# VITA-Group/mm-hand

Measured on AMD Instinct MI355X. Metric: 256x256 hand images/sec (G+D step), higher is better.
Workload: dtype f32; 1 GPU; RHD-shaped 256x256, per-GPU batch 32, fp32 (Winograd F(6x6,3x3) on the 3x3 stack), G(9 PATBlocks, ngf64)+D_PB+D_PP+L1/perceptual/GAN+Adam, --norm instance, dropout on; VGG19[:4] weights: random-init (seed 1234): NOT the reference's pretrained objective; global_batch=32, parallelism=dp1

## Files before the change

### mmhand_amd/csrc/common.h

```cpp
#pragma once
#include <hip/hip_runtime.h>
#include <cstdarg>
#include <cstdio>
#include <cstdint>
#include "../../include/mmhand_hip.h"

namespace mmh {

char* err_buf();
int fail(const char* fmt, ...);

inline int check_launch(const char* what) {
    hipError_t e = hipGetLastError();
    if (e != hipSuccess) return fail("%s: %s", what, hipGetErrorString(e));
    return 0;
}

inline hipStream_t as_stream(mmh_stream_t s) { return reinterpret_cast<hipStream_t>(s); }

inline int64_t cdiv(int64_t a, int64_t b) { return (a + b - 1) / b; }

int wino6_weights(const float* w, float* U, int Cin, int Cout, int flip_transpose, hipStream_t st);
int wino6_weights_multi(const long long* table, int n, long long total_blocks, hipStream_t st);
int wino6_input(const float* x, float* V, int B, int H, int W, int C, int reflect, int xcd, hipStream_t st);
int wino6_output(const float* M, float* y, const float* bias, int B, int H, int W, int C, int act, float* stats,
                 int fold, hipStream_t st);
int wino6_dy(const float* dy, float* Yh, int B, int H, int W, int C, hipStream_t st);
int wino6_input_normact(const float* x, float* V, int B, int H, int W, int C, int reflect, int xcd,
                        const float* scale, const float* shift, int groups, int relu, float drop_p,
                        const uint32_t* drows, hipStream_t st);
int wino6_input_dy_normbwd(const float* g, const float* x, float* V, float* Yh, int B, int H, int W, int C, int xcd,
                           int fold, const float* mean, const float* invstd, const float* gamma, const float* s1,
                           const float* s2, double count, const float* scale, const float* shift,
                           const uint32_t* drows, int groups, int relu, float drop_p, hipStream_t st);
int wino6_input_dy(const float* dy, float* V, float* Yh, int B, int H, int W, int C, int xcd, int fold,
                   hipStream_t st);
int wino6_dw(const float* dU, float* dw, int Cin, int Cout, int accumulate, hipStream_t st);
bool wgrad_lp16t_supported(const mmh_conv_desc* d);
int wgrad_lp16t_splits(const mmh_conv_desc* d);
int launch_wgrad_lp16t(const mmh_conv_desc* d, const void* x16, const void* dy16, float* slab, const void* zeros,
                       hipStream_t st);
bool dgrad_s2_halo_ok(const mmh_conv_desc* d, int dx_cs, int act);
int launch_dgrad_s2_halo(const mmh_conv_desc* d, const void* dy, const void* w, const void* bias, void* dx, int dx_cs,
                         int act, hipStream_t st);
extern int g_dgrad_s2_halo, g_dgrad_s2_dbg;
bool wgrad_s2_strip_ok(const mmh_conv_desc* d);
size_t wgrad_s2_strip_ws_bytes(const mmh_conv_desc* d);
int launch_wgrad_s2_strip(const mmh_conv_desc* d, const void* x, const void* dy, void* dw, void* ws, size_t ws_bytes,
                          int accumulate, hipStream_t st);
extern int g_wgrad_s2_strip;
bool stem_f32_ok(const mmh_conv_desc* d);
int stem_f32_stats_chunks(const mmh_conv_desc* d);
int launch_stem_f32(const mmh_conv_desc* d, const void* x, const void* w, const void* bias, void* y, int act, float* stats,
                    hipStream_t st);
extern int g_stem_f32, g_stem_f32_dbg, g_stem_f32_levels;
extern int g_stem_sparse;
extern int g_stem_sparse_flat;
void wgrad_flat_split(int Mrows, int N, int P, int& splits, int& pix_per_split);
bool wino_wgrad_dma_ok(int64_t tiles, int Cin, int Cout, int nbatch);
size_t wino_wgrad_dma_ws_bytes(int64_t tiles, int Cin, int Cout, int nbatch);
int launch_wino_wgrad_dma(const float* V, const float* Yh, int64_t tiles, int Cin, int Cout, int nbatch, float* ws, float* dU,
                          hipStream_t st);
extern int g_wino_wgrad_dma;
int launch_slab_reduce(const float* slab, float* dw, int64_t n4_total, int splits, int accumulate, int64_t n4, hipStream_t st);
bool conv_s2f_ok(const mmh_conv_desc* d, int mode);
bool conv_s1f_ok(const mmh_conv_desc* d, int mode);
int conv_s2f_stats_chunks(const mmh_conv_desc* d);
int launch_conv_s2f(const mmh_conv_desc* d, const void* x16, const void* w16, const void* bias, void* y, int y_is16, int act,
                    const void* zeros, hipStream_t st, float* stats = nullptr, int mode = 0);
bool conv_s2d_ok(const mmh_conv_desc* d, int mode);
int launch_conv_s2d(const mmh_conv_desc* d, const void* g16, const void* w16, const void* bias, void* dx, int dx_is16, int act,
                    const void* zeros, hipStream_t st);
extern int g_lp16_s2f;
extern int g_lp16_persist;
extern int g_slab_reduce_par;
extern int g_wino6_vec;
extern int g_lp16_shape;
extern int g_lp16_tap_inner;
extern int g_lp16_dbg;
extern int g_lp16_wgrad_ring;
extern int g_lp16_wgrad_s2;
extern int g_pw_v2;
extern int g_col_chunks, g_row_chunks;

}

#define MMH_REQUIRE(cond, ...)                      \
    do {                                            \
        if (!(cond)) return mmh::fail(__VA_ARGS__); \
    } while (0)
// ... 1 lines not shown
```

### mmhand_amd/csrc/conv_igemm.hip

```cpp
#include <algorithm>
#include <cstring>
#include "device_prims.h"

namespace {
using namespace mmh::dev;

typedef __bf16 bf16x4 __attribute__((ext_vector_type(4)));
typedef __bf16 bf16x2 __attribute__((ext_vector_type(2)));
typedef _Float16 f16x4 __attribute__((ext_vector_type(4)));
typedef _Float16 f16x2 __attribute__((ext_vector_type(2)));
__device__ __forceinline__ bf16x4 to_bf16x4(float4 v) {
    bf16x4 r;
    r[0] = (__bf16)v.x; r[1] = (__bf16)v.y; r[2] = (__bf16)v.z; r[3] = (__bf16)v.w;
    return r;
}
template <bool H16>
__device__ __forceinline__ bf16x4 to_lp4(float4 v) {
    if (H16) {
        f16x4 r;
        r[0] = (_Float16)v.x; r[1] = (_Float16)v.y; r[2] = (_Float16)v.z; r[3] = (_Float16)v.w;
        return __builtin_bit_cast(bf16x4, r);
    }
    return to_bf16x4(v);
}
// ... 2179 lines not shown

Gather fwd_gather(const mmh_conv_desc* d, const void* x) {
    Gather g{};
    g.src = static_cast<const float*>(x);
    g.src_bytes = (unsigned)((size_t)d->B * d->H * d->W * d->x_cs * sizeof(float));
    g.srcH = d->H; g.srcW = d->W; g.src_cs = (unsigned)d->x_cs;
    g.PH = d->Ho; g.PW = d->Wo;
    g.TH = d->kh; g.TW = d->kw;
    g.C4 = d->Cin / 4;
    g.ap_h = d->stride; g.at_h = 1; g.a0_h = -d->pad;
    g.ap_w = d->stride; g.at_w = 1; g.a0_w = -d->pad;
    g.shift = 0;
    g.reflect = d->pad_mode == MMH_PAD_REFLECT;
    return g;
}

int fprop_stats_chunks(const mmh_conv_desc* d) {
    if (mmh::stem_f32_ok(d)) return mmh::stem_f32_stats_chunks(d);
    const long long M = (long long)d->B * d->Ho * d->Wo;
    if (is16(d->dtype) || M % BM != 0 || d->Cout % 4 != 0) return 0;
    const int waves_m = d->Cout > 32 ? 2 : 4;
    return (int)(M / BM) * waves_m;
}

int do_fprop(const mmh_conv_desc* d, const void* x, const void* w, const void* bias, void* y,
             int act, hipStream_t st, float* stats = nullptr, const int* rect_pads = nullptr) {
    if (!rect_pads && mmh::stem_f32_ok(d) && (!stats || mmh::stem_f32_stats_chunks(d) > 0))
        return mmh::launch_stem_f32(d, x, w, bias, y, act, stats, st);
    ConvKP p{};
    p.stats = stats;
    p.g = fwd_gather(d, x);
    if (rect_pads) { p.g.a0_h = -rect_pads[0]; p.g.a0_w = -rect_pads[1]; }
    set_korder(p.g, p.nk, p.Kflat);
    p.w = static_cast<const float*>(w);
    p.w_bytes = (unsigned)((size_t)d->kh * d->kw * d->Cin * d->Cout * sizeof(float));
    p.out = static_cast<float*>(y);
    p.bias = static_cast<const float*>(bias);
    p.M = d->B * d->Ho * d->Wo;
    p.N = d->Cout;
    p.wCin = d->Cin; p.wCout = d->Cout;
    p.KW_true = d->kw; p.kh0 = 0; p.kw0 = 0; p.tstep = 1;
    p.out_linear = 1; p.out_cs = (unsigned)d->y_cs;
    p.OH = d->Ho; p.OW = d->Wo; p.o_p = 1;
    p.act = act;
    if (is16(d->dtype)) {
        p.h16 = d->dtype == MMH_FP16;
        if (d->Cin % 64 == 0) {
            p.wRows = d->Cout; p.wKper = d->Cin;
            p.w_bytes = (unsigned)((size_t)d->kh * d->kw * d->Cin * d->Cout * 2);
        } else {
            const int Kpad = (d->kh * d->kw * d->Cin + 63) / 64 * 64;
            p.flat16 = 1;
            p.wRows = d->Cout; p.wKper = Kpad;
            p.w_bytes = (unsigned)((size_t)d->Cout * Kpad * 2);
        }
        return launch_conv_bf16(p, st);
    }
    return launch_conv<false>(p, st);
}

int g_dgrad_s2_multi = 1;
template <int BN, int WM, int WN, int BMT = 128>
int launch_multi_t(MultiKP& mp, bool bf16, hipStream_t st);

int do_dgrad(const mmh_conv_desc* d, const void* dy, const void* w, const void* bias, void* dx,
             int dx_cs, int act, hipStream_t st) {
// ... 676 lines not shown
}

struct OptionEntry { const char* name; int* value; };
const OptionEntry* option_table(int* count) {
    static const OptionEntry table[] = {
        {"conv_dbuf", &g_conv_dbuf},
        {"conv_dbg", &g_conv_dbg},
        {"conv_cw", &g_conv_cw},
        {"conv_bn256", &g_conv_bn256},
        {"conv_levels", &g_conv_levels},
        {"dgrad_levels", &g_dgrad_levels},
        {"wino_bn256", &g_wino_bn256},
        {"conv_xcd", &g_conv_xcd},
        {"conv_xcd1", &g_conv_xcd1},
        {"conv_tall", &g_conv_tall},
        {"wgrad_slots", &g_wgrad_slots},
        {"wgrad_dbuf", &g_wgrad_dbuf},
        {"wgrad_bn256", &g_wgrad_bn256},
        {"wgrad_xcd", &g_wgrad_xcd},
        {"wino_wgrad_v2", &g_wino_wgrad_v2},
        {"wino_wgrad_occ", &g_wino_wgrad_occ},
        {"wino_gemm_v2", &g_wino_gemm_v2},
        {"wino_xcd", &g_wino_xcd},
        {"dgrad_s2_multi", &g_dgrad_s2_multi},
        {"wino6_vec", &mmh::g_wino6_vec},
        {"lp16_shape", &mmh::g_lp16_shape},
        {"lp16_s2f", &mmh::g_lp16_s2f},
        {"lp16_persist", &mmh::g_lp16_persist},
        {"lp16_tap_inner", &mmh::g_lp16_tap_inner},
        {"pw_v2", &mmh::g_pw_v2},
        {"col_chunks", &mmh::g_col_chunks},
        {"row_chunks", &mmh::g_row_chunks},
        {"dgrad_s2_halo", &mmh::g_dgrad_s2_halo},
        {"wgrad_s2_strip", &mmh::g_wgrad_s2_strip},
        {"stem_f32", &mmh::g_stem_f32},
        {"wino_wgrad_dma", &mmh::g_wino_wgrad_dma},
        {"stem_f32_dbg", &mmh::g_stem_f32_dbg},
        {"slab_reduce_par", &mmh::g_slab_reduce_par},
        {"dgrad_s2_dbg", &mmh::g_dgrad_s2_dbg},
        {"lp16_dbg", &mmh::g_lp16_dbg},
        {"lp16_wgrad_ring", &mmh::g_lp16_wgrad_ring},
        {"lp16_wgrad_s2", &mmh::g_lp16_wgrad_s2},
        {"border_bn64", &g_border_bn64},
        {"wino_gemm_occ", &g_wino_gemm_occ},
        {"wino_gemm_levels", &g_wino_gemm_levels},
        {"wino_gemm_bn", &g_wino_gemm_bn},
        {"wino_bf16_occ", &g_wino_bf16_occ},
        {"wino_bf16_bk", &g_wino_bf16_bk},
        {"wino_wgrad_bn256", &g_wino_wgrad_bn256},
        {"wino_wgrad_slots", &g_wino_wgrad_slots},
        {"stem_sparse", &mmh::g_stem_sparse},
        {"stem_sparse_flat", &mmh::g_stem_sparse_flat},
    };
    *count = (int)(sizeof(table) / sizeof(table[0]));
    return table;
}
const OptionEntry* find_option(const char* key) {
    int n = 0;
    const OptionEntry* t = option_table(&n);
    for (int i = 0; i < n; ++i)
        if (!strcmp(key, t[i].name)) return &t[i];
    return nullptr;
}

}

namespace mmh {
void wgrad_flat_split(int Mrows, int N, int P, int& splits, int& pix_per_split) {
    splits = wgrad_splits(Mrows, N, P);
    pix_per_split = wgrad_pix_per_split(P, splits, BK);
}
}

extern "C" {

int mmh_set_option(const char* key, int value) {
    MMH_REQUIRE(key != nullptr, "mmh_set_option: NULL key");
    const OptionEntry* e = find_option(key);
    if (!e) return mmh::fail("mmh_set_option: unknown key '%s'", key);
    if (e->value == &g_conv_levels) { g_conv_levels = value == 2 ? 2 : 1; mmh::g_stem_f32_levels = g_conv_levels; return 0; }
    if (e->value == &g_dgrad_levels) { g_dgrad_levels = value == 2 ? 2 : 1; return 0; }
    if (e->value == &mmh::g_col_chunks || e->value == &mmh::g_row_chunks)
        MMH_REQUIRE(value > 0, "mmh_set_option: '%s' needs a value > 0, got %d", key, value);
    *e->value = value;
    return 0;
// ... 506 lines not shown
```

### mmhand_amd/csrc/conv_thin.hip

```cpp
#include <algorithm>
#include "device_prims.h"

namespace {
using namespace mmh::dev;

constexpr int TW = 64, TH = 16;
constexpr int HC = TW + 6, HR = TH + 6;
constexpr unsigned OOBT = 0xFFFFFFF0u;

typedef float f2 __attribute__((ext_vector_type(2)));
typedef unsigned u4 __attribute__((ext_vector_type(4)));

struct ThinKP {
    const float* x;
    unsigned x_bytes;
    int B, H, W, Cin, x_cs;
    const float* w;
    const float* bias;
    float* y;
    int Ho, Wo, y_cs;
    int pad, reflect, act;
    int tiles_x, tiles_y;
    int x_lp;
};

__global__ void __launch_bounds__(256) thin_conv7_kernel(const ThinKP p) {
    __shared__ float4 xs[HR * HC];
    const int tid = threadIdx.x;
    const int lane = tid & 63, wave = tid >> 6;
    int t = blockIdx.x;
    const int tx = t % p.tiles_x; t /= p.tiles_x;
    const int ty = t % p.tiles_y;
    const int b = t / p.tiles_y;
    const int oh0 = ty * TH, ow0 = tx * TW;
    const __amdgpu_buffer_rsrc_t rs =
        __builtin_amdgcn_make_buffer_rsrc(const_cast<float*>(p.x), 0, p.x_bytes, 0x00020000);

    constexpr int NLD = (HR * HC + 255) / 256;
    unsigned soff[NLD];
#pragma unroll
    for (int i = 0; i < NLD; ++i) {
        const int idx = tid + 256 * i;
        const int r = idx / HC, c = idx - r * HC;
        int ih = oh0 + r - p.pad, iw = ow0 + c - p.pad;
        bool ok = idx < HR * HC;
        if (p.reflect) {
            ih = ih < 0 ? -ih : ih;
            iw = iw < 0 ? -iw : iw;
            ih = ih >= p.H ? 2 * (p.H - 1) - ih : ih;
            iw = iw >= p.W ? 2 * (p.W - 1) - iw : iw;
            ok = ok && ih >= 0 && iw >= 0 && ih < p.H && iw < p.W;
        } else {
            ok = ok && ih >= 0 && iw >= 0 && ih < p.H && iw < p.W;
        }
        soff[i] = ok ? (unsigned)(((b * p.H + ih) * p.W + iw) * p.x_cs) * (p.x_lp ? 2u : 4u) : OOBT;
    }

    f2 acc[4][2];
#pragma unroll
    for (int q = 0; q < 4; ++q) { acc[q][0] = (f2){0.f, 0.f}; acc[q][1] = (f2){0.f, 0.f}; }

    for (int c0 = 0; c0 < p.Cin; c0 += 4) {
        float4 st[NLD];
#pragma unroll
        for (int i = 0; i < NLD; ++i) {
            if (p.x_lp) {
                typedef unsigned u2 __attribute__((ext_vector_type(2)));
                const u2 v = __builtin_amdgcn_raw_buffer_load_b64(rs, soff[i] == OOBT ? OOBT : soff[i] + c0 * 2u, 0, 0);
                if (p.x_lp == 1) {
                    st[i] = make_float4(__uint_as_float(v[0] << 16), __uint_as_float(v[0] & 0xffff0000u),
                                        __uint_as_float(v[1] << 16), __uint_as_float(v[1] & 0xffff0000u));
                } else {
                    auto h = [](unsigned bits) { return (float)__builtin_bit_cast(_Float16, (unsigned short)bits); };
                    st[i] = make_float4(h(v[0] & 0xffffu), h(v[0] >> 16), h(v[1] & 0xffffu), h(v[1] >> 16));
                }
            } else {
                const u4 v = __builtin_amdgcn_raw_buffer_load_b128(rs, soff[i] == OOBT ? OOBT : soff[i] + c0 * 4u, 0, 0);
                st[i] = __builtin_bit_cast(float4, v);
            }
        }
        __syncthreads();
#pragma unroll
        for (int i = 0; i < NLD; ++i)
            if (tid + 256 * i < HR * HC) xs[tid + 256 * i] = st[i];
        __syncthreads();
        const float* wc = p.w + c0 * 4;
#pragma unroll 1
        for (int kw = 0; kw < 7; ++kw) {
            float4 xv[10];
// ... 5 lines not shown
                f2 w01[4], w23[4];
#pragma unroll
                for (int ci = 0; ci < 4; ++ci) {
                    w01[ci] = (f2){wt[ci * 4 + 0], wt[ci * 4 + 1]};
                    w23[ci] = (f2){wt[ci * 4 + 2], wt[ci * 4 + 3]};
                }
#pragma unroll
                for (int q = 0; q < 4; ++q) {
                    const float4 xx = xv[q + kh];
                    const float xc[4] = {xx.x, xx.y, xx.z, xx.w};
#pragma unroll
                    for (int ci = 0; ci < 4; ++ci) {
                        const f2 xb = (f2){xc[ci], xc[ci]};
                        acc[q][0] = __builtin_elementwise_fma(xb, w01[ci], acc[q][0]);
                        acc[q][1] = __builtin_elementwise_fma(xb, w23[ci], acc[q][1]);
                    }
                }
            }
        }
    }

    float bs[4] = {0.f, 0.f, 0.f, 0.f};
    if (p.bias) { bs[0] = p.bias[0]; bs[1] = p.bias[1]; bs[2] = p.bias[2]; bs[3] = p.bias[3]; }
    const int ow = ow0 + lane;
#pragma unroll
    for (int q = 0; q < 4; ++q) {
        const int oh = oh0 + wave * 4 + q;
        if (oh < p.Ho && ow < p.Wo) {
            float4 o;
            o.x = act_apply(acc[q][0].x + bs[0], p.act);
            o.y = act_apply(acc[q][0].y + bs[1], p.act);
            o.z = act_apply(acc[q][1].x + bs[2], p.act);
            o.w = act_apply(acc[q][1].y + bs[3], p.act);
            *reinterpret_cast<float4*>(p.y + ((size_t)(b * p.Ho + oh) * p.Wo + ow) * p.y_cs) = o;
        }
    }
}

__global__ void thin_flip_weights_kernel(const float* __restrict__ w, int wCin, int Cout, float* __restrict__ wq) {
    const int i = blockIdx.x * blockDim.x + threadIdx.x;
    if (i >= 49 * Cout * 4) return;
    const int j = i & 3;
    const int co = (i >> 2) % Cout;
    const int tap = (i >> 2) / Cout;
    const int kh = tap / 7, kw = tap - kh * 7;
    wq[i] = j < wCin ? w[(((6 - kh) * 7 + (6 - kw)) * wCin + j) * Cout + co] : 0.f;
}

__global__ void thin_reflect_fold_kernel(const float* __restrict__ dxp, float* __restrict__ dx, int B, int H, int W,
                                         int dx_cs, int p) {
    const long long total = (long long)B * H * W;
    long long i = (long long)blockIdx.x * blockDim.x + threadIdx.x;
    const long long stride = (long long)gridDim.x * blockDim.x;
    const int HP = H + 2 * p, WP = W + 2 * p;
    for (; i < total; i += stride) {
        const int w = (int)(i % W);
        const long long t = i / W;
        const int h = (int)(t % H);
        const int b = (int)(t / H);
        int hs[3], ws[3], nh = 0, nw = 0;
        hs[nh++] = h + p;
        if (h >= 1 && h <= p) hs[nh++] = p - h;
        if (h <= H - 2 && h >= H - 1 - p) hs[nh++] = 2 * (H - 1) - h + p;
        ws[nw++] = w + p;
        if (w >= 1 && w <= p) ws[nw++] = p - w;
        if (w <= W - 2 && w >= W - 1 - p) ws[nw++] = 2 * (W - 1) - w + p;
        float4 s = make_float4(0.f, 0.f, 0.f, 0.f);
        for (int a = 0; a < nh; ++a)
            for (int c = 0; c < nw; ++c) {
                const float4 v = *reinterpret_cast<const float4*>(dxp + ((size_t)(b * HP + hs[a]) * WP + ws[c]) * 4);
                s.x += v.x; s.y += v.y; s.z += v.z; s.w += v.w;
            }
        *reinterpret_cast<float4*>(dx + (size_t)i * dx_cs) = s;
    }
}

constexpr int WGW = 32;
constexpr int WGC = WGW + 6;

struct ThinWgKP {
    const float* x;
    unsigned x_bytes;
    const float* dy;
    unsigned dy_bytes;
    float* slab;
    int B, H, W, Cin, x_cs, dy_cs, reflect;
    int strips, chunks;
    int segs, seg_rows;
};

__global__ void __launch_bounds__(448) thin_wgrad7_kernel(const ThinWgKP p) {
    __shared__ float ring[8][WGC][64];
    __shared__ float4 dyrow[2][WGW];
    const int tid = threadIdx.x;
    const int lane = tid & 63, kh = tid >> 6;
    int t = blockIdx.x;
    const int chunk = t % p.chunks; t /= p.chunks;
    const int strip = t % p.strips; t /= p.strips;
    const int seg = t % p.segs;
    const int b = t / p.segs;
    const int r0 = seg * p.seg_rows, r1 = min(p.H, r0 + p.seg_rows);
    const int w0 = strip * WGW;
    const __amdgpu_buffer_rsrc_t rsx = __builtin_amdgcn_make_buffer_rsrc(const_cast<float*>(p.x), 0, p.x_bytes, 0x00020000);
    const __amdgpu_buffer_rsrc_t rsd = __builtin_amdgcn_make_buffer_rsrc(const_cast<float*>(p.dy), 0, p.dy_bytes, 0x00020000);

    constexpr int NF4 = WGC * 16;
    auto row_off = [&](int ir, int idx) -> unsigned {
        const int px = idx >> 4, c4 = idx & 15;
        int iw = w0 + px - 3;
        bool ok = idx < NF4;
        if (p.reflect) {
            ir = ir < 0 ? -ir : ir; ir = ir >= p.H ? 2 * (p.H - 1) - ir : ir;
            iw = iw < 0 ? -iw : iw; iw = iw >= p.W ? 2 * (p.W - 1) - iw : iw;
        }
        ok = ok && ir >= 0 && ir < p.H && iw >= 0 && iw < p.W;
        return ok ? (unsigned)(((b * p.H + ir) * p.W + iw) * p.x_cs + chunk * 64 + c4 * 4) * 4u : OOBT;
    };
    float4 st[2];
    float4 sd = make_float4(0.f, 0.f, 0.f, 0.f);
    auto load_row = [&](int ir, int orow) {
#pragma unroll
        for (int i = 0; i < 2; ++i) {
            const u4 v = __builtin_amdgcn_raw_buffer_load_b128(rsx, row_off(ir, tid + 448 * i), 0, 0);
            st[i] = __builtin_bit_cast(float4, v);
        }
        if (tid < WGW) {
            const int ow = w0 + tid;
            const unsigned off = (orow < p.H && ow < p.W) ? (unsigned)(((b * p.H + orow) * p.W + ow) * p.dy_cs) * 4u : OOBT;
            sd = __builtin_bit_cast(float4, __builtin_amdgcn_raw_buffer_load_b128(rsd, off, 0, 0));
        }
    };
    auto store_row = [&](int ir, int orow) {
        float* slot = &ring[(ir + 3) & 7][0][0];
#pragma unroll
        for (int i = 0; i < 2; ++i) {
            const int idx = tid + 448 * i;
            if (idx < NF4) *reinterpret_cast<float4*>(slot + (idx >> 4) * 64 + (idx & 15) * 4) = st[i];
        }
        if (tid < WGW) dyrow[orow & 1][tid] = sd;
    };

    f2 acc[7][2];
#pragma unroll
    for (int k = 0; k < 7; ++k) { acc[k][0] = (f2){0.f, 0.f}; acc[k][1] = (f2){0.f, 0.f}; }

    for (int ir = r0 - 3; ir <= r0 + 2; ++ir) { load_row(ir, p.H); store_row(ir, r0 + 1); }
    load_row(r0 + 3, r0);
    store_row(r0 + 3, r0);
    __syncthreads();
    for (int r = r0; r < r1; ++r) {
        if (r + 1 < r1) load_row(r + 4, r + 1);
        const float* xr = &ring[(r + kh) & 7][0][lane];
        float xv[WGC];
#pragma unroll
        for (int c = 0; c < WGC; ++c) xv[c] = xr[c * 64];
#pragma unroll
        for (int c = 0; c < WGW; ++c) {
            const float4 d4 = dyrow[r & 1][c];
            const f2 d01 = (f2){d4.x, d4.y}, d23 = (f2){d4.z, d4.w};
#pragma unroll
            for (int kw = 0; kw < 7; ++kw) {
                const f2 xb = (f2){xv[c + kw], xv[c + kw]};
                acc[kw][0] = __builtin_elementwise_fma(xb, d01, acc[kw][0]);
                acc[kw][1] = __builtin_elementwise_fma(xb, d23, acc[kw][1]);
            }
        }
        if (r + 1 < r1) store_row(r + 4, r + 1);
        __syncthreads();
    }
    float* out = p.slab + ((size_t)blockIdx.x * 49 + kh * 7) * 256 + lane * 4;
#pragma unroll
    for (int kw = 0; kw < 7; ++kw)
        *reinterpret_cast<float4*>(out + kw * 256) = make_float4(acc[kw][0].x, acc[kw][0].y, acc[kw][1].x, acc[kw][1].y);
}

__global__ void thin_wgrad_reduce_kernel(const float* __restrict__ slab, float* __restrict__ dw, int nbs, int chunks,
                                         int Cin, int accumulate) {
    const int i = blockIdx.x * blockDim.x + threadIdx.x;
    if (i >= 49 * Cin) return;
    const int tap = i / Cin, ci = i - tap * Cin;
    const int chunk = ci >> 6, cl = ci & 63;
    float4 s = make_float4(0.f, 0.f, 0.f, 0.f);
    for (int k = 0; k < nbs; ++k) {
        const float4 v = *reinterpret_cast<const float4*>(slab + (((size_t)(k * chunks + chunk) * 49 + tap) * 64 + cl) * 4);
        s.x += v.x; s.y += v.y; s.z += v.z; s.w += v.w;
    }
    float4* o = reinterpret_cast<float4*>(dw) + i;
    if (accumulate) { const float4 v = *o; s.x += v.x; s.y += v.y; s.z += v.z; s.w += v.w; }
    *o = s;
}

int launch_thin(ThinKP& p, hipStream_t st) {
    p.tiles_x = (p.Wo + TW - 1) / TW;
    p.tiles_y = (p.Ho + TH - 1) / TH;
    const long long blocks = (long long)p.B * p.tiles_x * p.tiles_y;
    MMH_REQUIRE(blocks > 0 && blocks < (1ll << 31), "thin conv: grid too large");
    hipLaunchKernelGGL(thin_conv7_kernel, dim3((unsigned)blocks), dim3(256), 0, st, p);
    return mmh::check_launch("thin_conv7_kernel");
}

bool thin_shape_ok(const mmh_conv_desc* d) {
    return d && d->kh == 7 && d->kw == 7 && d->stride == 1 && d->pad == 3 && d->dtype == MMH_F32 && d->B > 0 &&
           d->H > 3 && d->W > 3 && d->Ho == d->H && d->Wo == d->W;
}

}

extern "C" {

int mmh_conv7_thin_fprop(const mmh_conv_desc* d, const void* x, const void* w, const void* bias, void* y, int act,
                         mmh_stream_t s) {
    MMH_REQUIRE(thin_shape_ok(d), "mmh_conv7_thin_fprop: needs a 7x7 / stride 1 / pad 3 fp32 conv");
    MMH_REQUIRE(d->Cout == 4 && d->Cin % 4 == 0 && d->Cin > 0 && d->x_cs >= d->Cin && d->x_cs % 4 == 0 &&
                    d->y_cs >= 4 && d->y_cs % 4 == 0,
                "mmh_conv7_thin_fprop: needs Cout == 4 (3 padded to 4) and channel counts %% 4 == 0");
    MMH_REQUIRE(x && w && y, "mmh_conv7_thin_fprop: NULL buffer");
    const long long xb = (long long)d->B * d->H * d->W * d->x_cs * 4;
    MMH_REQUIRE(xb < (1ll << 32) - 64, "mmh_conv7_thin_fprop: input too large for 32-bit offsets");
    ThinKP p{};
    p.x = static_cast<const float*>(x); p.x_bytes = (unsigned)xb;
    p.B = d->B; p.H = d->H; p.W = d->W; p.Cin = d->Cin; p.x_cs = d->x_cs;
    p.w = static_cast<const float*>(w); p.bias = static_cast<const float*>(bias);
    p.y = static_cast<float*>(y); p.Ho = d->Ho; p.Wo = d->Wo; p.y_cs = d->y_cs;
    p.pad = 3; p.reflect = d->pad_mode == MMH_PAD_REFLECT; p.act = act;
    return launch_thin(p, mmh::as_stream(s));
}

size_t mmh_conv7_thin_dgrad_ws_bytes(const mmh_conv_desc* d) {
    if (!thin_shape_ok(d)) return 0;
// ... 44 lines not shown
static int thin_wg_segs(const mmh_conv_desc* d) {
    const long long base = (long long)d->B * ((d->W + WGW - 1) / WGW) * (d->Cin / 64);
    const long long want = (256 + base - 1) / base;
    return (int)std::max<long long>(1, std::min<long long>(want, d->H / 32));
}

size_t mmh_conv7_thin_wgrad_ws_bytes(const mmh_conv_desc* d) {
    if (!thin_shape_ok(d) || d->Cin % 64) return 0;
    const size_t nblk = (size_t)d->B * ((d->W + WGW - 1) / WGW) * (d->Cin / 64) * thin_wg_segs(d);
    return nblk * 49 * 64 * 4 * sizeof(float);
}

int mmh_conv7_thin_wgrad(const mmh_conv_desc* d, const void* x, const void* dy, void* dw, void* ws, size_t ws_bytes,
                         int accumulate, mmh_stream_t s) {
    MMH_REQUIRE(thin_shape_ok(d), "mmh_conv7_thin_wgrad: needs a 7x7 / stride 1 / pad 3 fp32 conv");
    MMH_REQUIRE(d->Cout == 4 && d->Cin % 64 == 0 && d->Cin > 0 && d->x_cs >= d->Cin && d->x_cs % 4 == 0 && d->y_cs >= 4 &&
                    d->y_cs % 4 == 0,
                "mmh_conv7_thin_wgrad: needs Cout == 4 and Cin %% 64 == 0");
    MMH_REQUIRE(x && dy && dw && ws && ws_bytes >= mmh_conv7_thin_wgrad_ws_bytes(d), "mmh_conv7_thin_wgrad: bad buffers");
    const long long xb = (long long)d->B * d->H * d->W * d->x_cs * 4, yb = (long long)d->B * d->H * d->W * d->y_cs * 4;
    MMH_REQUIRE(xb < (1ll << 32) - 64 && yb < (1ll << 32) - 64, "mmh_conv7_thin_wgrad: tensors too large for 32-bit offsets");
    hipStream_t st = mmh::as_stream(s);
    ThinWgKP p{};
    p.x = static_cast<const float*>(x); p.x_bytes = (unsigned)xb;
    p.dy = static_cast<const float*>(dy); p.dy_bytes = (unsigned)yb;
    p.slab = static_cast<float*>(ws);
    p.B = d->B; p.H = d->H; p.W = d->W; p.Cin = d->Cin; p.x_cs = d->x_cs; p.dy_cs = d->y_cs;
    p.reflect = d->pad_mode == MMH_PAD_REFLECT;
    p.strips = (d->W + WGW - 1) / WGW;
    p.chunks = d->Cin / 64;
    p.segs = thin_wg_segs(d);
    p.seg_rows = (d->H + p.segs - 1) / p.segs;
    const int nblk = d->B * p.segs * p.strips * p.chunks;
    hipLaunchKernelGGL(thin_wgrad7_kernel, dim3(nblk), dim3(448), 0, st, p);
    if (int rc = mmh::check_launch("thin_wgrad7_kernel")) return rc;
    const int n4 = 49 * d->Cin;
    hipLaunchKernelGGL(thin_wgrad_reduce_kernel, dim3((n4 + 255) / 256), dim3(256), 0, st, p.slab, static_cast<float*>(dw),
                       d->B * p.segs * p.strips, p.chunks, d->Cin, accumulate);
    return mmh::check_launch("thin_wgrad_reduce_kernel");
}

}
```

Measured before the change: 129.4 images/s.

## Add persistent XCD-aware MFMA kernel for stride-2 3x3 f32 forward convs

Adds a dedicated persistent kernel for the generator's stride-2 3x3 downsampling convolutions (64->128, 128->256) in fp32. It uses a three-stage LDS DMA pipeline, zero-line halo handling and fp32 32x32x2 MFMA, and fuses bias plus instance-norm statistics into the epilogue. The epilogue of each tile overlaps with loads for the next one. It replaces the generic implicit-GEMM path for these shapes when there is no activation. Risks are heavy LDS use at one block per CU and possible stats-layout mismatch with the generic path.

```diff
diff --git a/mmhand_amd/csrc/common.h b/mmhand_amd/csrc/common.h
--- a/mmhand_amd/csrc/common.h
+++ b/mmhand_amd/csrc/common.h
@@ -44,6 +44,10 @@
 int launch_dgrad_s2_halo(const mmh_conv_desc* d, const void* dy, const void* w, const void* bias, void* dx, int dx_cs,
                          int act, hipStream_t st);
 extern int g_dgrad_s2_halo, g_dgrad_s2_dbg;
+bool fprop_s2_ok(const mmh_conv_desc* d);
+int launch_fprop_s2(const mmh_conv_desc* d, const void* x, const void* w, const void* bias, void* y, float* stats,
+                    hipStream_t st);
+extern int g_fprop_s2_halo;
 bool wgrad_s2_strip_ok(const mmh_conv_desc* d);
 size_t wgrad_s2_strip_ws_bytes(const mmh_conv_desc* d);
 int launch_wgrad_s2_strip(const mmh_conv_desc* d, const void* x, const void* dy, void* dw, void* ws, size_t ws_bytes,
diff --git a/mmhand_amd/csrc/conv_igemm.hip b/mmhand_amd/csrc/conv_igemm.hip
--- a/mmhand_amd/csrc/conv_igemm.hip
+++ b/mmhand_amd/csrc/conv_igemm.hip
@@ -2235,6 +2235,8 @@
     p.g = fwd_gather(d, x);
     if (rect_pads) { p.g.a0_h = -rect_pads[0]; p.g.a0_w = -rect_pads[1]; }
     set_korder(p.g, p.nk, p.Kflat);
+    if (!rect_pads && act == MMH_ACT_NONE && g_conv_levels == 1 && p.g.chunk_major && p.g.cw == 2 && mmh::fprop_s2_ok(d))
+        return mmh::launch_fprop_s2(d, x, w, bias, y, stats, st);
     p.w = static_cast<const float*>(w);
     p.w_bytes = (unsigned)((size_t)d->kh * d->kw * d->Cin * d->Cout * sizeof(float));
     p.out = static_cast<float*>(y);
@@ -2977,6 +2979,7 @@
         {"col_chunks", &mmh::g_col_chunks},
         {"row_chunks", &mmh::g_row_chunks},
         {"dgrad_s2_halo", &mmh::g_dgrad_s2_halo},
+        {"fprop_s2_halo", &mmh::g_fprop_s2_halo},
         {"wgrad_s2_strip", &mmh::g_wgrad_s2_strip},
         {"stem_f32", &mmh::g_stem_f32},
         {"wino_wgrad_dma", &mmh::g_wino_wgrad_dma},
diff --git a/mmhand_amd/csrc/fprop_s2.hip b/mmhand_amd/csrc/fprop_s2.hip
--- /dev/null
+++ b/mmhand_amd/csrc/fprop_s2.hip
@@ -0,0 +1,275 @@
+#include <algorithm>
+#include <type_traits>
+#include "device_prims.h"
+
+namespace mmh { int g_fprop_s2_halo = 1; }
+
+namespace {
+using namespace mmh::dev;
+
+constexpr int NT = 512;
+constexpr int BMT = 128;
+constexpr int KP = 32;
+constexpr int NST = 3;
+constexpr int A_B = BMT * KP * 4;
+constexpr int b_bytes(int tn) { return KP * 128 * tn * 4; }
+constexpr int stage_bytes(int tn) { return A_B + b_bytes(tn); }
+constexpr int lds_bytes(int tn) { return NST * stage_bytes(tn); }
+
+__device__ __attribute__((aligned(128))) char g_zero_line[128];
+constexpr int wait_vm(int n) { return (n & 15) | ((n >> 4) << 14) | 0x0070; }
+template <int V> using IC = std::integral_constant<int, V>;
+
+struct FpropS2KP {
+    const float* x;
+    const float* w;
+    const float* bias;
+    float* y;
+    float* stats;
+    int H, W, Ho, Wo, x_cs, y_cs;
+    int tiles, per_xcd, slots;
+};
+
+template <int TN>
+__global__ void __launch_bounds__(NT, 1) fprop_s2_kernel(const FpropS2KP p) {
+    constexpr int N = 128 * TN, CIN = 64 * TN, SC = TN;
+    constexpr int B_B = b_bytes(TN), STAGE = stage_bytes(TN);
+    constexpr int BR = B_B / (NT * 16);
+    constexpr int NI = 2 + BR;
+    constexpr int CPR = N / 4;
+    constexpr int RPR = NT / CPR;
+    extern __shared__ __attribute__((aligned(1024))) char smem[];
+    const int tid = threadIdx.x;
+    const int lane = tid & 63, wave = __builtin_amdgcn_readfirstlane(tid >> 6);
+    const int l31 = lane & 31, h = lane >> 5;
+    const int wm = wave >> 2, wn = wave & 3;
+    const unsigned lds0 = lds_addr_of(smem);
+    const unsigned wdst = __builtin_amdgcn_readfirstlane(lds0 + (unsigned)wave * 1024u);
+    const int xcd = blockIdx.x & 7, slot = blockIdx.x >> 3;
+    const int t_end = min(p.tiles, (xcd + 1) * p.per_xcd);
+    int tile = xcd * p.per_xcd + slot;
+    if (tile >= t_end) return;
+
+    const int ncol = wn * 32 * TN + l31;
+    float bv[TN];
+#pragma unroll
+    for (int j = 0; j < TN; ++j) {
+        bv[j] = p.bias ? p.bias[ncol + 32 * j] : 0.f;
+        asm volatile("" : "+v"(bv[j]));
+    }
+
+    const int arow = tid >> 3;
+    const unsigned a_coff = (unsigned)(((tid & 7) ^ ((tid >> 4) & 7)) << 2);
+    const unsigned w_lane_off = (unsigned)(((tid / CPR) * N + ((tid % CPR) << 2)) * 4);
+    const int HoWo = p.Ho * p.Wo;
+    int ptile = tile, psc = 0, pkh = 0, pkw = 0, pj = 0;
+    int a_pix[2];
+    bool a_top[2], a_left[2];
+    auto set_ptile = [&]() {
+#pragma unroll
+        for (int rr = 0; rr < 2; ++rr) {
+            const int m = ptile * BMT + rr * 64 + arow;
+            const int b = m / HoWo;
+            const int rem = m - b * HoWo;
+            const int oh = rem / p.Wo, ow = rem - (rem / p.Wo) * p.Wo;
+            a_pix[rr] = (b * p.H + 2 * oh - 1) * p.W + 2 * ow - 1;
+            a_top[rr] = oh == 0;
+            a_left[rr] = ow == 0;
+        }
+    };
+    auto issue = [&](int stage) {
+        const bool live = ptile < t_end;
+        const int c0 = psc * 64 + pj * KP;
+        const unsigned dst = wdst + (unsigned)(stage * STAGE);
+#pragma unroll
+        for (int rr = 0; rr < 2; ++rr) {
+            const bool ok = live && !(pkh == 0 && a_top[rr]) && !(pkw == 0 && a_left[rr]);
+            const int pix = ok ? a_pix[rr] + pkh * p.W + pkw : 0;
+            const void* g = ok ? (const void*)(p.x + (size_t)pix * (size_t)p.x_cs + c0 + a_coff)
+                               : (const void*)(g_zero_line + (lane & 7) * 16);
+            lds_dma16(g, dst + (unsigned)(rr * NT * 16));
+        }
+        const float* src = p.w + (size_t)((pkh * 3 + pkw) * CIN + c0) * N;
+#pragma unroll
+        for (int rr = 0; rr < BR; ++rr) dma16_s(src + rr * RPR * N, w_lane_off, dst + (unsigned)(A_B + rr * NT * 16));
+        if (++pj == 2) {
+            pj = 0;
+            if (++pkw == 3) {
+                pkw = 0;
+                if (++pkh == 3) {
+                    pkh = 0;
+                    if (++psc == SC) { psc = 0; ptile += p.slots; set_ptile(); }
+                }
+            }
+        }
+    };
+
+    const unsigned a_lane = lds0 + (unsigned)((wm * 64 + l31) * (KP * 4)) + (unsigned)((h ^ ((l31 >> 1) & 7)) << 4);
+    const unsigned b_lane = lds0 + (unsigned)A_B + (unsigned)((h * 4 * N + ncol) * 4);
+    f32x16 acc[2][TN];
+
+    auto epilogue = [&](int t) {
+        float* const yo = p.y + (size_t)(t * BMT + wm * 64) * (size_t)p.y_cs + ncol;
+#pragma unroll
+        for (int i = 0; i < 2; ++i)
+#pragma unroll
+            for (int r = 0; r < 16; ++r) {
+                const int m = i * 32 + (r & 3) + 8 * (r >> 2) + 4 * h;
+#pragma unroll
+                for (int j = 0; j < TN; ++j) yo[(size_t)m * (size_t)p.y_cs + 32 * j] = acc[i][j][r] + bv[j];
+            }
+        if (p.stats) {
+            constexpr float CNT = 32.f;
+#pragma unroll
+            for (int j = 0; j < TN; ++j) {
+                const float b = bv[j];
+                float sum = 0.f;
+#pragma unroll
+                for (int i = 0; i < 2; ++i)
+#pragma unroll
+                    for (int r = 0; r < 16; ++r) sum += acc[i][j][r] + b;
+                const float mean_l = sum * (1.f / CNT);
+                float m2 = 0.f;
+#pragma unroll
+                for (int i = 0; i < 2; ++i)
+#pragma unroll
+                    for (int r = 0; r < 16; ++r) {
+                        const float dv = acc[i][j][r] + b - mean_l;
+                        m2 += dv * dv;
+                    }
+                const float mean_o = __shfl_xor(mean_l, 32, 64), m2_o = __shfl_xor(m2, 32, 64);
+                const float dm = mean_o - mean_l;
+                if (h == 0) {
+                    float* o = p.stats + ((size_t)(t * 2 + wm) * 3) * N + ncol + 32 * j;
+                    o[0] = 2.f * CNT;
+                    o[N] = mean_l + 0.5f * dm;
+                    o[2 * N] = m2 + m2_o + dm * dm * (0.5f * CNT);
+                }
+            }
+        }
+    };
+
+    int prev = -1;
+    auto phase = [&](auto phc, bool first) {
+        constexpr int ph = decltype(phc)::value;
+        constexpr int S = ph % NST, SN = (ph + 2) % NST;
+        asm volatile("" ::: "memory");
+        if (ph == 1 && first && prev >= 0) __builtin_amdgcn_s_waitcnt(wait_vm(0));
+        else __builtin_amdgcn_s_waitcnt(wait_vm(NI));
+        __builtin_amdgcn_s_barrier();
+        asm volatile("" ::: "memory");
+        issue(SN);
+        if (ph == 0 && first) {
+            if (prev >= 0) epilogue(prev);
+#pragma unroll
+            for (int i = 0; i < 2; ++i)
+#pragma unroll
+                for (int j = 0; j < TN; ++j)
+#pragma unroll
+                    for (int r = 0; r < 16; ++r) acc[i][j][r] = 0.f;
+        }
+        unsigned ab = a_lane + (unsigned)(S * STAGE), bb = b_lane + (unsigned)(S * STAGE);
+        asm volatile("" : "+v"(ab), "+v"(bb));
+        f32x4 af[2];
+        float bf[TN][4];
+#pragma unroll
+        for (int i = 0; i < 2; ++i) af[i] = lds_f4(ab, i * 32 * KP * 4);
+#pragma unroll
+        for (int j = 0; j < TN; ++j)
+#pragma unroll
+            for (int e = 0; e < 4; ++e) bf[j][e] = lds_f(bb, (e * N + 32 * j) * 4);
+#pragma unroll
+        for (int kg = 0; kg < 4; ++kg) {
+            f32x4 an[2];
+            float bn[TN][4];
+            if (kg + 1 < 4) {
+#pragma unroll
+                for (int i = 0; i < 2; ++i) an[i] = lds_f4(ab ^ (unsigned)((kg + 1) << 5), i * 32 * KP * 4);
+#pragma unroll
+                for (int j = 0; j < TN; ++j)
+#pragma unroll
+                    for (int e = 0; e < 4; ++e) bn[j][e] = lds_f(bb, (((kg + 1) * 8 + e) * N + 32 * j) * 4);
+            }
+#pragma unroll
+            for (int e = 0; e < 4; ++e)
+#pragma unroll
+                for (int i = 0; i < 2; ++i)
+#pragma unroll
+                    for (int j = 0; j < TN; ++j)
+                        acc[i][j] = __builtin_amdgcn_mfma_f32_32x32x2f32(af[i][e], bf[j][e], acc[i][j], 0, 0, 0);
+            if (kg + 1 < 4) {
+#pragma unroll
+                for (int i = 0; i < 2; ++i) af[i] = an[i];
+#pragma unroll
+                for (int j = 0; j < TN; ++j)
+#pragma unroll
+                    for (int e = 0; e < 4; ++e) bf[j][e] = bn[j][e];
+            }
+        }
+    };
+
+    set_ptile();
+    issue(0);
+    issue(1);
+    for (; tile < t_end; tile += p.slots) {
+        for (int sc = 0; sc < SC; ++sc)
+            for (int kh = 0; kh < 3; ++kh) {
+                const bool first = sc == 0 && kh == 0;
+                phase(IC<0>{}, first); phase(IC<1>{}, first); phase(IC<2>{}, first);
+                phase(IC<3>{}, first); phase(IC<4>{}, first); phase(IC<5>{}, first);
+            }
+        prev = tile;
+    }
+    epilogue(prev);
+    __builtin_amdgcn_s_waitcnt(wait_vm(0));
+}
+
+}
+
+namespace mmh {
+
+bool fprop_s2_ok(const mmh_conv_desc* d) {
+    return g_fprop_s2_halo && d->dtype == MMH_F32 && d->kh == 3 && d->kw == 3 && d->stride == 2 && d->pad == 1 &&
+           d->pad_mode == MMH_PAD_ZERO && ((d->Cin == 64 && d->Cout == 128) || (d->Cin == 128 && d->Cout == 256)) &&
+           d->H == 2 * d->Ho && d->W == 2 * d->Wo && ((long long)d->B * d->Ho * d->Wo) % BMT == 0 &&
+           d->x_cs >= d->Cin && d->x_cs % 4 == 0 && d->y_cs >= d->Cout &&
+           (long long)d->B * d->H * d->W * d->x_cs < (1ll << 31) && (long long)d->B * d->Ho * d->Wo * d->y_cs < (1ll << 31);
+}
+
+template <int TN>
+static int launch_t(const FpropS2KP& p, hipStream_t st) {
+    static int ready = -1;
+    if (ready != 0) {
+        hipError_t e = hipFuncSetAttribute(reinterpret_cast<const void*>(fprop_s2_kernel<TN>),
+                                           hipFuncAttributeMaxDynamicSharedMemorySize, lds_bytes(TN));
+        if (e != hipSuccess) return fail("fprop_s2: %s", hipGetErrorString(e));
+        ready = 0;
+    }
+    hipLaunchKernelGGL((fprop_s2_kernel<TN>), dim3(8 * p.slots), dim3(NT), lds_bytes(TN), st, p);
+    return check_launch("fprop_s2_kernel");
+}
+
+int launch_fprop_s2(const mmh_conv_desc* d, const void* x, const void* w, const void* bias, void* y, float* stats,
+                    hipStream_t st) {
+    FpropS2KP p{};
+    p.x = static_cast<const float*>(x);
+    p.w = static_cast<const float*>(w);
+    p.bias = static_cast<const float*>(bias);
+    p.y = static_cast<float*>(y);
+    p.stats = stats;
+    p.H = d->H; p.W = d->W; p.Ho = d->Ho; p.Wo = d->Wo; p.x_cs = d->x_cs; p.y_cs = d->y_cs;
+    p.tiles = (int)((long long)d->B * d->Ho * d->Wo / BMT);
+    p.per_xcd = (p.tiles + 7) / 8;
+    static int cus = 0;
+    if (!cus) {
+        int dev = 0;
+        hipDeviceProp_t prop;
+        if (hipGetDevice(&dev) != hipSuccess || hipGetDeviceProperties(&prop, dev) != hipSuccess)
+            return fail("fprop_s2: cannot query the device");
+        cus = prop.multiProcessorCount;
+    }
+    p.slots = std::max(1, std::min(cus / 8, p.per_xcd));
+    return d->Cin == 64 ? launch_t<1>(p, st) : launch_t<2>(p, st);
+}
+
+}
```

Measured after the change: 130.1 images/s (median of 6 runs). About the same (+0.6%).

## Use 4x4x1 f32 MFMA broadcast for thin 7x7 conv fprop and wgrad

Applied to the files above, without the earlier changes.

Adds MFMA variants of the thin 7x7 Cout=4 convolution forward and weight-gradient kernels. Both use the 4x4x1 f32 matrix instruction in broadcast mode to replace scalar FMA chains. The forward kernel restructures staging to 16-channel groups with a register prefetch of the next group's weights and input. The new path is on by default behind a thin_mfma option, but the forward MFMA path runs only for fp32 input. It raises register pressure through the 49-entry weight double buffer and triples shared memory in fprop, and these kernels are a small part of the full G+D step.

```diff
diff --git a/mmhand_amd/csrc/common.h b/mmhand_amd/csrc/common.h
--- a/mmhand_amd/csrc/common.h
+++ b/mmhand_amd/csrc/common.h
@@ -56,6 +56,7 @@
 extern int g_stem_f32, g_stem_f32_dbg, g_stem_f32_levels;
 extern int g_stem_sparse;
 extern int g_stem_sparse_flat;
+extern int g_thin_mfma;
 void wgrad_flat_split(int Mrows, int N, int P, int& splits, int& pix_per_split);
 bool wino_wgrad_dma_ok(int64_t tiles, int Cin, int Cout, int nbatch);
 size_t wino_wgrad_dma_ws_bytes(int64_t tiles, int Cin, int Cout, int nbatch);
diff --git a/mmhand_amd/csrc/conv_igemm.hip b/mmhand_amd/csrc/conv_igemm.hip
--- a/mmhand_amd/csrc/conv_igemm.hip
+++ b/mmhand_amd/csrc/conv_igemm.hip
@@ -2996,6 +2996,7 @@
         {"wino_wgrad_slots", &g_wino_wgrad_slots},
         {"stem_sparse", &mmh::g_stem_sparse},
         {"stem_sparse_flat", &mmh::g_stem_sparse_flat},
+        {"thin_mfma", &mmh::g_thin_mfma},
     };
     *count = (int)(sizeof(table) / sizeof(table[0]));
     return table;
diff --git a/mmhand_amd/csrc/conv_thin.hip b/mmhand_amd/csrc/conv_thin.hip
--- a/mmhand_amd/csrc/conv_thin.hip
+++ b/mmhand_amd/csrc/conv_thin.hip
@@ -1,5 +1,8 @@
 #include <algorithm>
+#include <type_traits>
 #include "device_prims.h"
+
+namespace mmh { int g_thin_mfma = 1; }
 
 namespace {
 using namespace mmh::dev;
@@ -10,6 +13,16 @@
 
 typedef float f2 __attribute__((ext_vector_type(2)));
 typedef unsigned u4 __attribute__((ext_vector_type(4)));
+typedef float f4 __attribute__((ext_vector_type(4)));
+
+template <int ABID>
+__device__ __forceinline__ f4 mfma_bcast(float a, float b, f4 c) {
+    return __builtin_amdgcn_mfma_f32_4x4x1f32(a, b, c, 4, ABID, 0);
+}
+template <int I, int N, class F>
+__device__ __forceinline__ void static_for(F&& f) {
+    if constexpr (I < N) { f(std::integral_constant<int, I>{}); static_for<I + 1, N>(f); }
+}
 
 struct ThinKP {
     const float* x;
@@ -24,6 +37,28 @@
     int x_lp;
 };
 
+constexpr int NLD = (HR * HC + 255) / 256;
+template <int PT, int N>
+__device__ __forceinline__ void thin_stage_offsets(const ThinKP& p, int tid, int b, int oh0, int ow0, unsigned (&soff)[N]) {
+#pragma unroll
+    for (int i = 0; i < N; ++i) {
+        const int idx = (tid + 256 * i) / PT;
+        const int r = idx / HC, c = idx - r * HC;
+        int ih = oh0 + r - p.pad, iw = ow0 + c - p.pad;
+        bool ok = idx < HR * HC;
+        if (p.reflect) {
+            ih = ih < 0 ? -ih : ih;
+            iw = iw < 0 ? -iw : iw;
+            ih = ih >= p.H ? 2 * (p.H - 1) - ih : ih;
+            iw = iw >= p.W ? 2 * (p.W - 1) - iw : iw;
+            ok = ok && ih >= 0 && iw >= 0 && ih < p.H && iw < p.W;
+        } else {
+            ok = ok && ih >= 0 && iw >= 0 && ih < p.H && iw < p.W;
+        }
+        soff[i] = ok ? (unsigned)(((b * p.H + ih) * p.W + iw) * p.x_cs) * (p.x_lp ? 2u : 4u) : OOBT;
+    }
+}
+
 __global__ void __launch_bounds__(256) thin_conv7_kernel(const ThinKP p) {
     __shared__ float4 xs[HR * HC];
     const int tid = threadIdx.x;
@@ -35,26 +70,8 @@
     const int oh0 = ty * TH, ow0 = tx * TW;
     const __amdgpu_buffer_rsrc_t rs =
         __builtin_amdgcn_make_buffer_rsrc(const_cast<float*>(p.x), 0, p.x_bytes, 0x00020000);
-
-    constexpr int NLD = (HR * HC + 255) / 256;
     unsigned soff[NLD];
-#pragma unroll
-    for (int i = 0; i < NLD; ++i) {
-        const int idx = tid + 256 * i;
-        const int r = idx / HC, c = idx - r * HC;
-        int ih = oh0 + r - p.pad, iw = ow0 + c - p.pad;
-        bool ok = idx < HR * HC;
-        if (p.reflect) {
-            ih = ih < 0 ? -ih : ih;
-            iw = iw < 0 ? -iw : iw;
-            ih = ih >= p.H ? 2 * (p.H - 1) - ih : ih;
-            iw = iw >= p.W ? 2 * (p.W - 1) - iw : iw;
-            ok = ok && ih >= 0 && iw >= 0 && ih < p.H && iw < p.W;
-        } else {
-            ok = ok && ih >= 0 && iw >= 0 && ih < p.H && iw < p.W;
-        }
-        soff[i] = ok ? (unsigned)(((b * p.H + ih) * p.W + iw) * p.x_cs) * (p.x_lp ? 2u : 4u) : OOBT;
-    }
+    thin_stage_offsets<1>(p, tid, b, oh0, ow0, soff);
 
     f2 acc[4][2];
 #pragma unroll
@@ -126,6 +143,103 @@
             o.y = act_apply(acc[q][0].y + bs[1], p.act);
             o.z = act_apply(acc[q][1].x + bs[2], p.act);
             o.w = act_apply(acc[q][1].y + bs[3], p.act);
+            *reinterpret_cast<float4*>(p.y + ((size_t)(b * p.Ho + oh) * p.Wo + ow) * p.y_cs) = o;
+        }
+    }
+}
+
+__device__ __forceinline__ float thin_load_w(__amdgpu_buffer_rsrc_t rsw, unsigned byte_off) {
+    return __builtin_bit_cast(float, __builtin_amdgcn_raw_buffer_load_b32(rsw, byte_off, 0, 0));
+}
+
+constexpr int NLD16 = (HR * HC * 4 + 255) / 256;
+
+__global__ void __launch_bounds__(256) thin_conv7_mfma_kernel(const ThinKP p) {
+    __shared__ float4 xs[4][HR * HC];
+    const int tid = threadIdx.x;
+    const int lane = tid & 63, wave = tid >> 6;
+    int t = blockIdx.x;
+    const int tx = t % p.tiles_x; t /= p.tiles_x;
+    const int ty = t % p.tiles_y;
+    const int b = t / p.tiles_y;
+    const int oh0 = ty * TH, ow0 = tx * TW;
+    const __amdgpu_buffer_rsrc_t rs =
+        __builtin_amdgcn_make_buffer_rsrc(const_cast<float*>(p.x), 0, p.x_bytes, 0x00020000);
+    const __amdgpu_buffer_rsrc_t rsw =
+        __builtin_amdgcn_make_buffer_rsrc(const_cast<float*>(p.w), 0, 49 * p.Cin * 16, 0x00020000);
+    unsigned soff[NLD16];
+    thin_stage_offsets<4>(p, tid, b, oh0, ow0, soff);
+    const int cu = tid & 3;
+
+    float4 st[NLD16];
+    float wn[49], wc[49];
+    auto load_stage = [&](int g) {
+#pragma unroll
+        for (int k = 0; k < 49; ++k) wn[k] = thin_load_w(rsw, (unsigned)((k * p.Cin + g) * 4 + lane) * 4u);
+        const bool cok = g + 4 * cu < p.Cin;
+#pragma unroll
+        for (int i = 0; i < NLD16; ++i)
+            st[i] = __builtin_bit_cast(float4, __builtin_amdgcn_raw_buffer_load_b128(
+                                                   rs, soff[i] == OOBT || !cok ? OOBT : soff[i] + (g + 4 * cu) * 4u, 0, 0));
+    };
+
+    f4 acc[4];
+#pragma unroll
+    for (int q = 0; q < 4; ++q) acc[q] = (f4){0.f, 0.f, 0.f, 0.f};
+    const float4* xw = &xs[0][wave * 4 * HC + lane];
+    load_stage(0);
+    for (int g = 0; g < p.Cin; g += 16) {
+#pragma unroll
+        for (int i = 0; i < NLD16; ++i)
+            if ((tid + 256 * i) >> 2 < HR * HC) xs[cu][(tid + 256 * i) >> 2] = st[i];
+#pragma unroll
+        for (int k = 0; k < 49; ++k) wc[k] = wn[k];
+        __syncthreads();
+        if (g + 16 < p.Cin) load_stage(g + 16);
+        float4 xv[2][10];
+#pragma unroll
+        for (int r = 0; r < 10; ++r) xv[0][r] = xw[r * HC];
+        static_for<0, 4>([&](auto u) {
+            constexpr int U = decltype(u)::value;
+            if (g + 4 * U < p.Cin)
+                static_for<0, 7>([&](auto k) {
+                    constexpr int KW = decltype(k)::value, CUR = (U * 7 + KW) & 1;
+                    constexpr int NU = KW == 6 ? U + 1 : U, NKW = KW == 6 ? 0 : KW + 1;
+                    if constexpr (NU < 4) {
+#pragma unroll
+                        for (int r = 0; r < 10; ++r) xv[CUR ^ 1][r] = xw[NU * HR * HC + r * HC + NKW];
+                    }
+                    __builtin_amdgcn_sched_barrier(0);
+#pragma unroll
+                    for (int kh = 0; kh < 7; ++kh) {
+                        const float w = wc[kh * 7 + KW];
+#pragma unroll
+                        for (int q = 0; q < 4; ++q) acc[q] = mfma_bcast<U * 4 + 0>(w, xv[CUR][q + kh].x, acc[q]);
+#pragma unroll
+                        for (int q = 0; q < 4; ++q) acc[q] = mfma_bcast<U * 4 + 1>(w, xv[CUR][q + kh].y, acc[q]);
+#pragma unroll
+                        for (int q = 0; q < 4; ++q) acc[q] = mfma_bcast<U * 4 + 2>(w, xv[CUR][q + kh].z, acc[q]);
+#pragma unroll
+                        for (int q = 0; q < 4; ++q) acc[q] = mfma_bcast<U * 4 + 3>(w, xv[CUR][q + kh].w, acc[q]);
+                    }
+                    __builtin_amdgcn_sched_barrier(0);
+                });
+        });
+        __syncthreads();
+    }
+
+    float bs[4] = {0.f, 0.f, 0.f, 0.f};
+    if (p.bias) { bs[0] = p.bias[0]; bs[1] = p.bias[1]; bs[2] = p.bias[2]; bs[3] = p.bias[3]; }
+    const int ow = ow0 + lane;
+#pragma unroll
+    for (int q = 0; q < 4; ++q) {
+        const int oh = oh0 + wave * 4 + q;
+        if (oh < p.Ho && ow < p.Wo) {
+            float4 o;
+            o.x = act_apply(acc[q][0] + bs[0], p.act);
+            o.y = act_apply(acc[q][1] + bs[1], p.act);
+            o.z = act_apply(acc[q][2] + bs[2], p.act);
+            o.w = act_apply(acc[q][3] + bs[3], p.act);
             *reinterpret_cast<float4*>(p.y + ((size_t)(b * p.Ho + oh) * p.Wo + ow) * p.y_cs) = o;
         }
     }
@@ -183,7 +297,8 @@
     int segs, seg_rows;
 };
 
-__global__ void __launch_bounds__(448) thin_wgrad7_kernel(const ThinWgKP p) {
+template <bool MFMA>
+__device__ __forceinline__ void thin_wgrad7_body(const ThinWgKP& p) {
     __shared__ float ring[8][WGC][64];
     __shared__ float4 dyrow[2][WGW];
     const int tid = threadIdx.x;
@@ -234,9 +349,9 @@
         if (tid < WGW) dyrow[orow & 1][tid] = sd;
     };
 
-    f2 acc[7][2];
-#pragma unroll
-    for (int k = 0; k < 7; ++k) { acc[k][0] = (f2){0.f, 0.f}; acc[k][1] = (f2){0.f, 0.f}; }
+    f4 acc[7];
+#pragma unroll
+    for (int k = 0; k < 7; ++k) acc[k] = (f4){0.f, 0.f, 0.f, 0.f};
 
     for (int ir = r0 - 3; ir <= r0 + 2; ++ir) { load_row(ir, p.H); store_row(ir, r0 + 1); }
     load_row(r0 + 3, r0);
@@ -248,15 +363,25 @@
         float xv[WGC];
 #pragma unroll
         for (int c = 0; c < WGC; ++c) xv[c] = xr[c * 64];
-#pragma unroll
-        for (int c = 0; c < WGW; ++c) {
-            const float4 d4 = dyrow[r & 1][c];
-            const f2 d01 = (f2){d4.x, d4.y}, d23 = (f2){d4.z, d4.w};
-#pragma unroll
-            for (int kw = 0; kw < 7; ++kw) {
-                const f2 xb = (f2){xv[c + kw], xv[c + kw]};
-                acc[kw][0] = __builtin_elementwise_fma(xb, d01, acc[kw][0]);
-                acc[kw][1] = __builtin_elementwise_fma(xb, d23, acc[kw][1]);
+        if constexpr (MFMA) {
+            const float* dr = reinterpret_cast<const float*>(&dyrow[r & 1][0]);
+            const float dreg[WGW / 16] = {dr[lane], dr[64 + lane]};
+            static_for<0, WGW>([&](auto cc) {
+                constexpr int c = decltype(cc)::value;
+#pragma unroll
+                for (int kw = 0; kw < 7; ++kw) acc[kw] = mfma_bcast<c % 16>(dreg[c / 16], xv[c + kw], acc[kw]);
+            });
+        } else {
+#pragma unroll
+            for (int c = 0; c < WGW; ++c) {
+                const float4 d4 = dyrow[r & 1][c];
+                const f2 d01 = (f2){d4.x, d4.y}, d23 = (f2){d4.z, d4.w};
+#pragma unroll
+                for (int kw = 0; kw < 7; ++kw) {
+                    const f2 xb = (f2){xv[c + kw], xv[c + kw]};
+                    acc[kw].lo = __builtin_elementwise_fma(xb, d01, acc[kw].lo);
+                    acc[kw].hi = __builtin_elementwise_fma(xb, d23, acc[kw].hi);
+                }
             }
         }
         if (r + 1 < r1) store_row(r + 4, r + 1);
@@ -265,8 +390,11 @@
     float* out = p.slab + ((size_t)blockIdx.x * 49 + kh * 7) * 256 + lane * 4;
 #pragma unroll
     for (int kw = 0; kw < 7; ++kw)
-        *reinterpret_cast<float4*>(out + kw * 256) = make_float4(acc[kw][0].x, acc[kw][0].y, acc[kw][1].x, acc[kw][1].y);
-}
+        *reinterpret_cast<float4*>(out + kw * 256) = make_float4(acc[kw][0], acc[kw][1], acc[kw][2], acc[kw][3]);
+}
+
+__global__ void __launch_bounds__(448) thin_wgrad7_kernel(const ThinWgKP p) { thin_wgrad7_body<false>(p); }
+__global__ void __launch_bounds__(448) thin_wgrad7_mfma_kernel(const ThinWgKP p) { thin_wgrad7_body<true>(p); }
 
 __global__ void thin_wgrad_reduce_kernel(const float* __restrict__ slab, float* __restrict__ dw, int nbs, int chunks,
                                          int Cin, int accumulate) {
@@ -289,6 +417,10 @@
     p.tiles_y = (p.Ho + TH - 1) / TH;
     const long long blocks = (long long)p.B * p.tiles_x * p.tiles_y;
     MMH_REQUIRE(blocks > 0 && blocks < (1ll << 31), "thin conv: grid too large");
+    if (mmh::g_thin_mfma && p.x_lp == 0) {
+        hipLaunchKernelGGL(thin_conv7_mfma_kernel, dim3((unsigned)blocks), dim3(256), 0, st, p);
+        return mmh::check_launch("thin_conv7_mfma_kernel");
+    }
     hipLaunchKernelGGL(thin_conv7_kernel, dim3((unsigned)blocks), dim3(256), 0, st, p);
     return mmh::check_launch("thin_conv7_kernel");
 }
@@ -399,8 +531,9 @@
     p.segs = thin_wg_segs(d);
     p.seg_rows = (d->H + p.segs - 1) / p.segs;
     const int nblk = d->B * p.segs * p.strips * p.chunks;
-    hipLaunchKernelGGL(thin_wgrad7_kernel, dim3(nblk), dim3(448), 0, st, p);
-    if (int rc = mmh::check_launch("thin_wgrad7_kernel")) return rc;
+    if (mmh::g_thin_mfma) hipLaunchKernelGGL(thin_wgrad7_mfma_kernel, dim3(nblk), dim3(448), 0, st, p);
+    else hipLaunchKernelGGL(thin_wgrad7_kernel, dim3(nblk), dim3(448), 0, st, p);
+    if (int rc = mmh::check_launch(mmh::g_thin_mfma ? "thin_wgrad7_mfma_kernel" : "thin_wgrad7_kernel")) return rc;
     const int n4 = 49 * d->Cin;
     hipLaunchKernelGGL(thin_wgrad_reduce_kernel, dim3((n4 + 255) / 256), dim3(256), 0, st, p.slab, static_cast<float*>(dw),
                        d->B * p.segs * p.strips, p.chunks, d->Cin, accumulate);
```

New measurement: 128.6 images/s before, 129.3 images/s after, median of 6. No clear change (+0.5%).
